# klausondrag/FOSVOS

Hardware: AMD Instinct MI355X
Metric: online fine-tune frames/sec (854x480) (higher is better)
Workload: dtype bf16; 1 GPU; OSVOS_VGG train_online one-shot fine-tune: 1x3x480x854 frame per step, fwd + class-balanced BCE + bwd, fused SGD step every 5 steps (BASELINE.json configs[1]); batch=1, avg_grad_every_n=5, activations=bf16 NHWC, fp32 accumulate, fp32 master weights, parallelism=single GPU

## Files before the change

### fosvos_amd/csrc/common.hpp

```cpp
#pragma once
#include <hip/hip_runtime.h>
#include <stdarg.h>
#include <algorithm>
#include <stdint.h>
#include <stdio.h>
#include <stdlib.h>
#include <string.h>

#include "../../include/fosvos_hip.h"

namespace fosvos {

extern thread_local char g_err[512];

inline int fail(int code, const char *fmt, ...) __attribute__((format(printf, 2, 3)));
inline int fail(int code, const char *fmt, ...) {
    va_list ap;
    va_start(ap, fmt);
    vsnprintf(g_err, sizeof(g_err), fmt, ap);
    va_end(ap);
    return code;
}

#define FOSVOS_HIP_CHECK(expr)                                                                         \
// ... 47 lines not shown
int wgrad_queue_reduce(const float *slabs, const float *bias_part, float *dw, float *db, int S, int S_bias, int64_t E_real,
                       int64_t E_pad, int Co, int Cor, int accumulate, WgradReduceTable *reduce, int device, void *stream);
struct HeadBwdArgs {
    const float *const *side;
    const int *hs, *ws;
    const float *const *filt, *const *filt1;
    const float *dsn_w, *fuse_w, *d_fused;
    const float *const *d_side_out;
    uint16_t *const *d_side;
    float *d_fuse_w, *d_fuse_b, *d_dsn_w, *d_dsn_b;
    int N, H, W, accumulate;
    void *workspace;
    size_t workspace_bytes;
    int device;
    int filt_uniform;
};
int head_bwd_check(const HeadBwdArgs &a);
int head_bwd_scale(const HeadBwdArgs &a, int s, void *stream);
int head_bwd_finish(const HeadBwdArgs &a, void *stream);

}
constexpr int kFosvosVggEvents = 25, kFosvosResnetEvents = 12;
struct fosvos_ctx {
    uint32_t magic;
    int device;
    hipEvent_t vgg_ev[kFosvosVggEvents];
    hipEvent_t resnet_ev[kFosvosResnetEvents];
    bool buckets_recorded;
};
constexpr uint32_t kFosvosCtxMagic = 0x58544346u;
namespace fosvos {
inline int ctx_check(const fosvos_ctx *ctx, const char *who) {
    FOSVOS_REQUIRE(ctx != nullptr, FOSVOS_E_ARG, "%s: null context (fosvos_ctx_create)", who);
    FOSVOS_REQUIRE(ctx->magic == kFosvosCtxMagic, FOSVOS_E_ARG, "%s: not a live fosvos_ctx", who);
    return FOSVOS_OK;
}

#ifdef FOSVOS_LAB_BUILD
inline const char *lab_env(const char *name) { return getenv(name); }
#else
inline const char *lab_env(const char *) { return nullptr; }
#endif
inline int lab_env_int(const char *name, int dflt) {
    const char *e = lab_env(name);
    return e ? atoi(e) : dflt;
}

bool conv_pp_applicable(int N, int H, int W, int in_ch, int out_ch);
int conv_pp_workgroups();
int conv_pp_forward(const uint16_t *x, const uint16_t *w_packed, const float *bias, uint16_t *y, uint16_t *y_pool, int N,
                    int H, int W, int Cin_pad, int Cout, int Co_pad, bool relu, hipStream_t st,
                    const uint8_t *mask_bits = nullptr, uint32_t *codes = nullptr);

bool conv3x3_pool_codes_applicable(int N, int H, int W, int Ci, int Co);

inline int64_t cdiv(int64_t a, int64_t b) { return (a + b - 1) / b; }
inline int roundup(int a, int b) { return (a + b - 1) / b * b; }

typedef uint16_t bf16_t;
typedef __attribute__((ext_vector_type(8))) __bf16 bf16x8;
typedef __attribute__((ext_vector_type(4))) float f32x4;
typedef __attribute__((ext_vector_type(4))) short s16x4;
typedef unsigned int u32x4 __attribute__((__vector_size__(16)));

__device__ __forceinline__ uint16_t f2bf(float f) {
    __bf16 b = (__bf16)f;
    return __builtin_bit_cast(uint16_t, b);
}
__device__ __forceinline__ float bf2f(uint16_t v) { return __uint_as_float(((uint32_t)v) << 16); }
__device__ __forceinline__ uint4 repack8(const float (&f)[8]) {
    uint4 v;
    v.x = __builtin_amdgcn_perm(__float_as_uint(f[1]), __float_as_uint(f[0]), 0x07060302u);
    v.y = __builtin_amdgcn_perm(__float_as_uint(f[3]), __float_as_uint(f[2]), 0x07060302u);
    v.z = __builtin_amdgcn_perm(__float_as_uint(f[5]), __float_as_uint(f[4]), 0x07060302u);
    v.w = __builtin_amdgcn_perm(__float_as_uint(f[7]), __float_as_uint(f[6]), 0x07060302u);
    return v;
}
typedef float fosvos_f32x2 __attribute__((ext_vector_type(2)));
typedef __bf16 fosvos_bf16x2 __attribute__((ext_vector_type(2)));
__device__ __forceinline__ uint32_t pack2bf(float lo, float hi) {
    const fosvos_f32x2 v = {lo, hi};
    return __builtin_bit_cast(uint32_t, __builtin_convertvector(v, fosvos_bf16x2));
}
__device__ __forceinline__ float relu_f(float v) { return __int_as_float(max(__float_as_int(v), 0)); }
__device__ __forceinline__ void unpack8(const uint4 &v, float (&f)[8]) {
    f[0] = __uint_as_float(v.x << 16);
    f[1] = __uint_as_float(v.x & 0xffff0000u);
    f[2] = __uint_as_float(v.y << 16);
    f[3] = __uint_as_float(v.y & 0xffff0000u);
    f[4] = __uint_as_float(v.z << 16);
    f[5] = __uint_as_float(v.z & 0xffff0000u);
    f[6] = __uint_as_float(v.w << 16);
    f[7] = __uint_as_float(v.w & 0xffff0000u);
}
__device__ __forceinline__ uint4 pack8(const float (&f)[8]) {
    uint4 v;
    v.x = pack2bf(f[0], f[1]);
    v.y = pack2bf(f[2], f[3]);
    v.z = pack2bf(f[4], f[5]);
    v.w = pack2bf(f[6], f[7]);
    return v;
}

typedef short fosvos_i16x2 __attribute__((ext_vector_type(2)));
typedef unsigned short fosvos_u16x2 __attribute__((ext_vector_type(2)));
__device__ __forceinline__ uint32_t keep_where_pos_bf16x2(uint32_t f, uint32_t m) {
// ... 92 lines not shown
```

### fosvos_amd/csrc/conv_igemm.hip

```cpp
#include <stdlib.h>

#include "common.hpp"

using namespace fosvos;

namespace {

constexpr unsigned kReluAfterAdd = 0x100u;
constexpr unsigned kSubsample2 = 0x200u;
constexpr unsigned kNoSplitK = 0x400u;

struct ConvArgs {
    const uint16_t *x;
    const uint16_t *w;
    const float *bias;
    const uint16_t *relu_src;
    const uint8_t *relu_bits;
    const uint16_t *addend;
    void *y;
    uint16_t *y_pool;
    const uint16_t *unpool_g;
    int N, H, W, Cin, Cout, Co_pad;
    int tiles_x, tiles_y;
    unsigned flags;
// ... 759 lines not shown
    if ((flags & ~FOSVOS_CONV_RELU) || addend) return false;
    if (dgrad) {
        if (lab_env_int("FOSVOS_PP_DGRAD", 1) == 0 || lab_env_int("FOSVOS_PP", -1) == 0) return false;
    } else {
        static const int mode = lab_env_int("FOSVOS_PP", -1);
        if (mode == 0) return false;
    }
    return conv_pp_applicable(N, H, W, roundup(in_ch, 32), out_ch);
}

int check_common(const void *x, const void *w, const void *y, int N, int H, int W, int in_ch, int out_ch,
                 const char *who) {
    FOSVOS_REQUIRE(x && w && y, FOSVOS_E_ARG, "%s: null pointer", who);
    FOSVOS_REQUIRE(N > 0 && H > 0 && W > 0 && in_ch > 0 && out_ch > 0, FOSVOS_E_SHAPE, "%s: bad shape N=%d H=%d W=%d in=%d out=%d",
                   who, N, H, W, in_ch, out_ch);
    FOSVOS_REQUIRE(out_ch % 16 == 0, FOSVOS_E_SHAPE, "%s: output channels %d not a multiple of 16", who, out_ch);
    FOSVOS_REQUIRE((int64_t)H * W * roundup(in_ch, 32) * 2 < 0x7fffffffLL && (int64_t)H * W * out_ch * 4 < 0x7fffffffLL,
                   FOSVOS_E_SHAPE, "%s: one image exceeds 2^31 bytes", who);
    return FOSVOS_OK;
}
}

extern "C" size_t fosvos_conv3x3_workspace_bytes(int N, int H, int W, int in_ch, int out_ch) {
    if (N <= 0 || H <= 0 || W <= 0 || in_ch <= 0 || out_ch <= 0 || (out_ch % 64 != 0 && out_ch != 16)) return 0;
    return make_plan(N, H, W, in_ch, out_ch).workspace_bytes;
}

extern "C" int fosvos_conv3x3_plan(int N, int H, int W, int in_ch, int out_ch, fosvos_conv3x3_plan_info *out) {
    FOSVOS_REQUIRE(out, FOSVOS_E_ARG, "conv3x3_plan: null output");
    FOSVOS_REQUIRE(N > 0 && H > 0 && W > 0 && in_ch > 0 && out_ch > 0 && (out_ch % 64 == 0 || out_ch == 32 || out_ch == 16),
                   FOSVOS_E_SHAPE, "conv3x3_plan: bad shape N=%d H=%d W=%d in=%d out=%d", N, H, W, in_ch, out_ch);
    const ConvPlan p = make_plan(N, H, W, in_ch, out_ch);
    out->k_splits = p.k_splits;
    out->persistent = 0;
    return with_tile(p.tile, [&](auto t) {
        out->tile_h = t.TH; out->tile_w = t.TW; out->tile_co = t.BN;
        out->workgroups = (int)(cdiv(W, t.TW) * cdiv(H, t.TH) * N * (out_ch / t.BN));
        return FOSVOS_OK;
    });
}

extern "C" int fosvos_conv3x3_fwd_plan(int N, int H, int W, int in_ch, int out_ch, unsigned flags,
                                       fosvos_conv3x3_plan_info *out) {
    if (int rc = fosvos_conv3x3_plan(N, H, W, in_ch, out_ch, out)) return rc;
    if (takes_pp(N, H, W, in_ch, out_ch, flags)) {
        out->tile_h = 8; out->tile_w = 32; out->tile_co = 64;
        out->k_splits = 1;
        out->workgroups = conv_pp_workgroups();
        out->persistent = 1;
    }
    return FOSVOS_OK;
}

extern "C" int fosvos_conv3x3_fwd(const uint16_t *x, const uint16_t *w_packed, const float *bias, void *y, int N, int H,
                                  int W, int Ci, int Co, unsigned flags, void *workspace, size_t workspace_bytes,
                                  int device, void *stream) {
    if (int rc = check_common(x, w_packed, y, N, H, W, Ci, Co, "conv3x3_fwd")) return rc;
    FOSVOS_REQUIRE((flags & ~(FOSVOS_CONV_RELU | FOSVOS_CONV_OUT_F32)) == 0, FOSVOS_E_ARG, "conv3x3_fwd: unknown flags 0x%x", flags);
    FOSVOS_ENTER(device);
    if (takes_pp(N, H, W, Ci, Co, flags))
        return conv_pp_forward(x, w_packed, bias, (uint16_t *)y, nullptr, N, H, W, roundup(Ci, 32), Co, roundup(Co, 16),
                               (flags & FOSVOS_CONV_RELU) != 0, (hipStream_t)stream);
    ConvArgs a = conv_args(x, w_packed, y, N, H, W, Ci, Co);
    a.bias = bias; a.flags = flags;
    return dispatch(a, Ci, workspace, workspace_bytes, (hipStream_t)stream);
}

extern "C" int fosvos_conv3x3_fwd_add(const uint16_t *x, const uint16_t *w_packed, const float *bias,
                                      const uint16_t *addend, void *y, int N, int H, int W, int Ci, int Co,
                                      unsigned flags, void *workspace, size_t workspace_bytes, int device,
                                      void *stream) {
    if (int rc = check_common(x, w_packed, y, N, H, W, Ci, Co, "conv3x3_fwd_add")) return rc;
    FOSVOS_REQUIRE((flags & ~(FOSVOS_CONV_RELU | FOSVOS_CONV_OUT_F32)) == 0, FOSVOS_E_ARG, "conv3x3_fwd_add: unknown flags 0x%x",
                   flags);
    FOSVOS_REQUIRE(Co % 64 == 0 || Co == 32 || (Co == 16 && !addend), FOSVOS_E_SHAPE,
                   "conv3x3_fwd_add: Co=%d must be 32 or a multiple of 64 (16 without an addend)", Co);
    FOSVOS_REQUIRE(!(flags & FOSVOS_CONV_OUT_F32) || (Co == 16 && !addend), FOSVOS_E_ARG,
                   "conv3x3_fwd_add: fp32 output is the 16-channel side_prep form");
    FOSVOS_ENTER(device);
    ConvArgs a = conv_args(x, w_packed, y, N, H, W, Ci, Co);
    a.bias = bias; a.addend = addend;
    a.flags = kNoSplitK | (addend ? ((flags & FOSVOS_CONV_RELU) ? kReluAfterAdd : 0u) : flags);
    return dispatch(a, Ci, workspace, workspace_bytes, (hipStream_t)stream);
}

extern "C" int fosvos_conv3x3_s2_fwd(const uint16_t *x, const uint16_t *w_packed, const float *bias, uint16_t *y, int N,
                                     int H, int W, int Ci, int Co, unsigned flags, void *workspace, size_t workspace_bytes,
                                     int device, void *stream) {
    if (int rc = check_common(x, w_packed, y, N, H, W, Ci, Co, "conv3x3_s2_fwd")) return rc;
    FOSVOS_REQUIRE((flags & ~FOSVOS_CONV_RELU) == 0, FOSVOS_E_ARG, "conv3x3_s2_fwd: unknown flags 0x%x", flags);
    FOSVOS_REQUIRE(Co % 64 == 0 || Co == 32, FOSVOS_E_SHAPE, "conv3x3_s2_fwd: Co=%d must be 32 or a multiple of 64", Co);
    FOSVOS_ENTER(device);
    ConvArgs a = conv_args(x, w_packed, y, N, H, W, Ci, Co);
    a.bias = bias; a.flags = flags | kSubsample2 | kNoSplitK;
    return dispatch(a, Ci, workspace, workspace_bytes, (hipStream_t)stream);
}

extern "C" int fosvos_conv3x3_fwd_pool(const uint16_t *x, const uint16_t *w_packed, const float *bias, uint16_t *y,
                                       uint16_t *y_pool, int N, int H, int W, int Ci, int Co, unsigned flags,
                                       void *workspace, size_t workspace_bytes, int device, void *stream) {
    if (int rc = check_common(x, w_packed, y, N, H, W, Ci, Co, "conv3x3_fwd_pool")) return rc;
    FOSVOS_REQUIRE(y_pool, FOSVOS_E_ARG, "conv3x3_fwd_pool: null pooled output");
    FOSVOS_REQUIRE((flags & ~FOSVOS_CONV_RELU) == 0, FOSVOS_E_ARG, "conv3x3_fwd_pool: unknown flags 0x%x", flags);
    FOSVOS_REQUIRE(Co % 64 == 0, FOSVOS_E_SHAPE, "conv3x3_fwd_pool: Co=%d must be a multiple of 64", Co);
    if ((flags & FOSVOS_CONV_RELU) && takes_pp(N, H, W, Ci, Co, flags)) {
        FOSVOS_ENTER(device);
        return conv_pp_forward(x, w_packed, bias, y, y_pool, N, H, W, roundup(Ci, 32), Co, roundup(Co, 16), true,
                               (hipStream_t)stream);
    }
    if (make_plan(N, H, W, Ci, Co).k_splits > 1) {
        if (int rc = fosvos_conv3x3_fwd(x, w_packed, bias, y, N, H, W, Ci, Co, flags, workspace, workspace_bytes, device, stream))
            return rc;
        return fosvos_maxpool2x2_ceil_fwd(y, y_pool, N, H, W, Co, device, stream);
    }
    FOSVOS_ENTER(device);
// ... 77 lines not shown
```

### fosvos_amd/fosvos_hip/__init__.py

```python
from __future__ import annotations

import ctypes
import os
import threading
from ctypes import POINTER, c_char_p, c_float, c_int, c_int64, c_size_t, c_uint, c_void_p

_HERE = os.path.dirname(os.path.abspath(__file__))
PKG_ROOT = os.path.dirname(_HERE)
LIB_PATH = os.environ.get("FOSVOS_HIP_LIB") or os.path.join(PKG_ROOT, "lib", "libfosvos_hip.so")
HEADER_PATH = os.path.join(os.path.dirname(PKG_ROOT), "include", "fosvos_hip.h")

ABI_VERSION = 34
CONV_RELU = 1
CONV_OUT_F32 = 2
VGG_COMPACT_STAGE1 = 1


class FosvosHipError(RuntimeError):
    pass


class SgdEntry(ctypes.Structure):
    _fields_ = [("param", c_void_p), ("grad", c_void_p), ("momentum_buf", c_void_p), ("numel", c_int64),
                ("lr", c_float), ("weight_decay", c_float)]
# ... 24 lines not shown
    _fields_ = [("total", c_size_t), ("stage_h", c_int * 5), ("stage_w", c_int * 5),
                ("act", _Z13), ("gact", _Z13), ("act_bytes", _Z13),
                ("pooled", _Z4), ("gpooled", _Z4), ("pooled_bytes", _Z4),
                ("side", _Z4), ("side_bytes", _Z4), ("dside", _Z4), ("dside_bytes", _Z4),
                ("bits0", c_size_t), ("bits0_bytes", c_size_t),
                ("ws", c_size_t), ("ws_bytes", c_size_t), ("hws", c_size_t), ("hws_bytes", c_size_t),
                ("wsa_conv", _Z13), ("wsa_conv_bytes", _Z13), ("wsa_side", _Z4), ("wsa_side_bytes", _Z4)]


class Conv3x3PlanInfo(ctypes.Structure):
    _fields_ = [("tile_h", c_int), ("tile_w", c_int), ("tile_co", c_int), ("k_splits", c_int), ("workgroups", c_int),
                ("persistent", c_int)]


class Conv2dPlanInfo(ctypes.Structure):
    _fields_ = [("cob", c_int), ("threads", c_int), ("slices", c_int), ("workgroups", c_int), ("mfma_frag_blocks", c_int),
                ("mfma_workgroups", c_int)]


class ProfileRecord(ctypes.Structure):
    _fields_ = [("name", ctypes.c_char * 96), ("launches", c_int), ("ms", ctypes.c_double), ("flops", ctypes.c_double)]


class PackEntry(ctypes.Structure):
    _fields_ = [("w", c_void_p), ("w_fwd", c_void_p), ("w_dgrad", c_void_p), ("Co", c_int), ("Ci", c_int)]



class Conv2dDesc(ctypes.Structure):
    _fields_ = [("w_packed", c_void_p), ("bias", c_void_p), ("Ci", c_int), ("Co", c_int), ("k", c_int), ("stride", c_int),
                ("kind", c_int)]


class ResnetBlock(ctypes.Structure):
    _fields_ = [("conv", Conv2dDesc * 3), ("n_convs", c_int), ("has_down", c_int), ("down", Conv2dDesc)]


class ResnetNet(ctypes.Structure):
    _fields_ = [("first_w", c_void_p), ("first_b", c_void_p), ("first_co", c_int), ("first_fp32_math", c_int), ("first_unfused", c_int),
                ("blocks_per_stage", c_int * 4),
                ("blocks", POINTER(ResnetBlock)), ("side", Conv2dDesc * 4), ("filt", c_void_p * 4),
                ("filt1", c_void_p * 4), ("stride", c_int * 4), ("dsn_w", c_void_p), ("dsn_b", c_void_p),
                ("fuse_b", c_void_p)]

SIGNATURES = {
    "fosvos_abi_version": (c_int, []),
    "fosvos_last_error": (c_char_p, []),
    "fosvos_build_arch": (c_char_p, []),
    "fosvos_ctx_create": (c_int, [c_int, POINTER(c_void_p)]),
    "fosvos_ctx_destroy": (c_int, [c_void_p]),
    "fosvos_ctx_device": (c_int, [c_void_p]),
    "fosvos_conv3x3_plan": (c_int, [c_int, c_int, c_int, c_int, c_int, POINTER(Conv3x3PlanInfo)]),
    "fosvos_conv3x3_fwd_plan": (c_int, [c_int, c_int, c_int, c_int, c_int, ctypes.c_uint, POINTER(Conv3x3PlanInfo)]),
    "fosvos_conv3x3_first_plan": (c_int, [c_int, c_int, c_int, POINTER(c_int), POINTER(c_int)]),
    "fosvos_nchw_f32_to_nhwc_bf16": (c_int, [c_void_p, c_void_p, c_int, c_int, c_int, c_int, c_int, c_int, c_void_p]),
    "fosvos_nhwc_bf16_to_nchw_f32": (c_int, [c_void_p, c_void_p, c_int, c_int, c_int, c_int, c_int, c_int, c_void_p]),
    "fosvos_nhwc_f32_to_nchw_f32": (c_int, [c_void_p, c_void_p, c_int, c_int, c_int, c_int, c_int, c_void_p]),
    "fosvos_nchw_f32_to_nhwc_f32": (c_int, [c_void_p, c_void_p, c_int, c_int, c_int, c_int, c_int, c_void_p]),
    "fosvos_pack_conv3x3_weights": (c_int, [c_void_p, c_int, c_int, c_void_p, c_void_p, c_int, c_void_p]),
    "fosvos_packed_weight_elems": (c_size_t, [c_int, c_int]),
    "fosvos_pack_conv3x3_weights_multi": (c_int, [POINTER(PackEntry), c_int, c_int, c_void_p]),
    "fosvos_conv3x3_first_fwd": (c_int, [c_void_p, c_void_p, c_void_p, c_void_p, c_void_p, c_int, c_int, c_int, c_int, c_int,
                                         c_void_p]),
    "fosvos_conv3x3_dgrad_bits": (c_int, [c_void_p, c_void_p, c_void_p, c_void_p, c_void_p, c_int, c_int, c_int, c_int,
                                          c_int, c_void_p, c_size_t, c_int, c_void_p]),
    "fosvos_conv3x3_dgrad_unpool": (c_int, [c_void_p, c_void_p, c_void_p, c_void_p, c_void_p, c_int, c_int, c_int, c_int,
                                            c_int, c_void_p, c_size_t, c_int, c_void_p]),
    "fosvos_conv3x3_first_wgrad": (c_int, [c_void_p, c_void_p, c_void_p, c_void_p, c_int, c_int, c_int, c_int,
                                           c_void_p, c_size_t, c_int, c_void_p]),
    "fosvos_conv3x3_first_wgrad_workspace_bytes": (c_size_t, [c_int, c_int, c_int, c_int]),
    "fosvos_conv3x3_fwd": (c_int, [c_void_p, c_void_p, c_void_p, c_void_p, c_int, c_int, c_int, c_int, c_int, c_uint,
                                   c_void_p, c_size_t, c_int, c_void_p]),
    "fosvos_conv3x3_fwd_pool": (c_int, [c_void_p, c_void_p, c_void_p, c_void_p, c_void_p, c_int, c_int, c_int, c_int,
                                        c_int, c_uint, c_void_p, c_size_t, c_int, c_void_p]),
    "fosvos_conv3x3_workspace_bytes": (c_size_t, [c_int, c_int, c_int, c_int, c_int]),
    "fosvos_conv3x3_dgrad": (c_int, [c_void_p, c_void_p, c_void_p, c_void_p, c_void_p, c_int, c_int, c_int, c_int,
                                     c_int, c_void_p, c_size_t, c_int, c_void_p]),
    "fosvos_conv3x3_wgrad": (c_int, [c_void_p, c_void_p, c_void_p, c_void_p, c_int, c_int, c_int, c_int, c_int, c_int,
                                     c_void_p, c_size_t, c_int, c_void_p]),
    "fosvos_conv3x3_wgrad_slabs": (c_int, [c_void_p, c_void_p, c_int, c_int, c_int, c_int, c_int, c_int, c_void_p, c_size_t,
                                           c_int, c_void_p]),
    "fosvos_conv3x3_wgrad_reduce": (c_int, [c_void_p, c_void_p, c_int, c_int, c_int, c_int, c_int, c_int, c_void_p,
                                            c_size_t, c_int, c_void_p]),
    "fosvos_conv3x3_wgrad_workspace_bytes": (c_size_t, [c_int, c_int, c_int, c_int, c_int]),
    "fosvos_maxpool2x2_ceil_fwd": (c_int, [c_void_p, c_void_p, c_int, c_int, c_int, c_int, c_int, c_void_p]),
    "fosvos_maxpool2x2_ceil_bwd": (c_int, [c_void_p, c_void_p, c_void_p, c_int, c_int, c_int, c_int, c_int, c_int,
                                           c_void_p]),
    "fosvos_head_fwd": (c_int, [POINTER(c_void_p), POINTER(c_int), POINTER(c_int), POINTER(c_void_p),
                                POINTER(c_void_p), c_void_p, c_void_p, c_void_p, c_void_p, c_void_p,
                                POINTER(c_void_p), c_int, c_int, c_int, c_int, c_int, c_void_p]),
    "fosvos_head_bwd": (c_int, [POINTER(c_void_p), POINTER(c_int), POINTER(c_int), POINTER(c_void_p),
                                POINTER(c_void_p), c_void_p, c_void_p, c_void_p, POINTER(c_void_p),
                                POINTER(c_void_p), c_void_p, c_void_p, c_void_p, c_void_p, c_int, c_int, c_int, c_int,
                                c_void_p, c_size_t, c_int, c_void_p]),
    "fosvos_head_bwd_workspace_bytes": (c_size_t, [c_int, c_int, c_int]),
    "fosvos_cbce_loss": (c_int, [c_void_p, c_void_p, c_int64, c_int, c_float, c_void_p, c_void_p, c_void_p, c_size_t,
                                 c_int, c_void_p]),
    "fosvos_cbce_workspace_bytes": (c_size_t, [c_int64]),
    "fosvos_cbce_loss_frames": (c_int, [c_void_p, c_void_p, c_int64, c_int, c_int, c_float, c_void_p, c_void_p, c_void_p,
                                        c_size_t, c_int, c_void_p]),
    "fosvos_cbce_loss_frames_parts": (c_int, [c_void_p, c_void_p, c_int64, c_int, c_int, c_float, c_void_p, c_void_p,
                                              c_void_p, c_size_t, c_int, c_int, c_void_p]),
    "fosvos_cbce_multi_workspace_bytes": (c_size_t, [c_int64, c_int, c_int]),
    "fosvos_cbce_loss_frames_multi": (c_int, [POINTER(c_void_p), c_void_p, c_int64, c_int, c_int, c_int, POINTER(c_float),
                                              c_void_p, POINTER(c_void_p), c_void_p, c_size_t, c_int, c_int, c_void_p]),
    "fosvos_cbce_loss_batch_counts": (c_int, [c_void_p, c_void_p, c_int64, c_int, c_float, c_void_p, c_void_p, c_void_p,
# ... 195 lines not shown
```

### fosvos_amd/fosvos_hip/ops.py

```python
from __future__ import annotations

import ctypes
import math
from typing import List, Optional, Sequence, Tuple

import torch

from . import CONV_OUT_F32, CONV_RELU, check, int_array4, lib, limits, ptr_array4

_BF16 = torch.bfloat16
_F32 = torch.float32


def _need(t: torch.Tensor, dtype, what: str, dtype_error=TypeError) -> torch.Tensor:
    if not t.is_cuda:
        raise RuntimeError(f"{what}: tensor must live on the GPU (the HIP path has no CPU fallback)")
    if t.dtype != dtype:
        raise dtype_error(f"{what}: expected {dtype}, got {t.dtype}")
    if not t.is_contiguous():
        raise ValueError(f"{what}: tensor must be contiguous")
    return t


def _ctx(t: torch.Tensor) -> Tuple[int, int]:
# ... 139 lines not shown
        if (kh, kw) != (3, 3) or w.device != ws[0].device:
            raise ValueError("pack_conv3x3_weights_multi: 3x3 kernels on one device only")
        fwd = torch.empty(L.fosvos_packed_weight_elems(co, ci), dtype=_BF16, device=w.device)
        dgr = torch.empty(L.fosvos_packed_weight_elems(ci, co), dtype=_BF16, device=w.device)
        arr[i].w, arr[i].w_fwd, arr[i].w_dgrad, arr[i].Co, arr[i].Ci = w.data_ptr(), fwd.data_ptr(), dgr.data_ptr(), co, ci
        out.append((fwd, dgr))
        nbytes += w.numel() * 4 + 2 * (fwd.numel() + dgr.numel())
    _launch("pack_conv3x3_weights_multi", ws[0], arr, len(ws), record="pack_weights", nbytes=nbytes)
    return out


def conv3x3_first_fwd(frame: torch.Tensor, w: torch.Tensor, b: torch.Tensor, want_bits: bool = False):
    _need(frame, _F32, "conv3x3_first_fwd frame"); _need(w, _F32, "conv3x3_first_fwd weight"); _need(b, _F32, "conv3x3_first_fwd bias")
    n, c, h, wd = frame.shape
    if c != 3 or tuple(w.shape[1:]) != (3, 3, 3):
        raise ValueError("conv3x3_first_fwd: expects a 3-channel frame and [Co,3,3,3] weights")
    co = w.shape[0]
    y = torch.empty((n, h, wd, co), dtype=_BF16, device=frame.device)
    bits = torch.empty((n, h, wd, co // 8), dtype=torch.uint8, device=frame.device) if want_bits else None
    _launch("conv3x3_first_fwd", frame, frame.data_ptr(), w.data_ptr(), b.data_ptr(), y.data_ptr(), _p(bits), n, h, wd, co,
            record="conv1_1_fwd", flops=2.0 * n * h * wd * 27 * co, nbytes=n * h * wd * (12 + 2 * co))
    return (y, bits) if want_bits else y


def conv3x3_first_wgrad(frame: torch.Tensor, dy: torch.Tensor) -> Tuple[torch.Tensor, torch.Tensor]:
    _need(frame, _F32, "conv3x3_first_wgrad frame"); _need(dy, _BF16, "conv3x3_first_wgrad dy")
    n, c, h, wd = frame.shape
    co = dy.shape[3]
    if tuple(dy.shape[:3]) != (n, h, wd):
        raise ValueError("conv3x3_first_wgrad: dy shape mismatch")
    L = lib()
    dw = torch.empty((co, 3, 3, 3), dtype=_F32, device=frame.device)
    db = torch.empty((co,), dtype=_F32, device=frame.device)
    ws, wsn = _WS.get(L.fosvos_conv3x3_first_wgrad_workspace_bytes(n, h, wd, co), frame.device)
    _launch("conv3x3_first_wgrad", frame, frame.data_ptr(), dy.data_ptr(), dw.data_ptr(), db.data_ptr(), n, h, wd, co, ws, wsn,
            record="conv1_1_wgrad", flops=2.0 * n * h * wd * 27 * co, nbytes=n * h * wd * (12 + 2 * co))
    return dw, db


def conv3x3_plan(n: int, h: int, w: int, in_ch: int, out_ch: int) -> dict:
    from . import Conv3x3PlanInfo
    info = Conv3x3PlanInfo()
    check(lib().fosvos_conv3x3_plan(n, h, w, in_ch, out_ch, ctypes.byref(info)), "conv3x3_plan")
    return {"tile": (info.tile_h, info.tile_w, info.tile_co), "k_splits": info.k_splits, "workgroups": info.workgroups,
            "persistent": bool(info.persistent)}


def conv3x3_fwd_plan(n: int, h: int, w: int, in_ch: int, out_ch: int, relu: bool = True) -> dict:
    from . import Conv3x3PlanInfo
    info = Conv3x3PlanInfo()
    check(lib().fosvos_conv3x3_fwd_plan(n, h, w, in_ch, out_ch, CONV_RELU if relu else 0, ctypes.byref(info)), "conv3x3_fwd_plan")
    return {"tile": (info.tile_h, info.tile_w, info.tile_co), "k_splits": info.k_splits, "workgroups": info.workgroups,
            "persistent": bool(info.persistent)}


def vgg_arena_layout(n: int, h: int, w: int) -> dict:
    from . import VggArenaLayout
    info = VggArenaLayout()
    check(lib().fosvos_vgg_arena_layout(n, h, w, ctypes.byref(info)), "vgg_arena_layout")
    out = {}
    for name, _ in VggArenaLayout._fields_:
        v = getattr(info, name)
        out[name] = list(v) if isinstance(v, ctypes.Array) else int(v)
    return out


def conv3x3_first_plan(n: int, h: int, w: int) -> Tuple[int, int]:
    tiles, wgs = ctypes.c_int(), ctypes.c_int()
    check(lib().fosvos_conv3x3_first_plan(n, h, w, ctypes.byref(tiles), ctypes.byref(wgs)), "conv3x3_first_plan")
    return tiles.value, wgs.value


def conv3x3_fwd(x: torch.Tensor, w_packed: torch.Tensor, bias: Optional[torch.Tensor], ci: int, co: int,
                relu: bool = True, out_f32: bool = False) -> torch.Tensor:
    _need(x, _BF16, "conv3x3_fwd x"); _need(w_packed, _BF16, "conv3x3_fwd packed weight")
    n, h, wd, cx = x.shape
    if cx != _ru(ci, 32):
        raise ValueError(f"conv3x3_fwd: x has {cx} channels, expected {_ru(ci, 32)} (Ci={ci} padded to 32)")
    L = lib()
    if w_packed.numel() != L.fosvos_packed_weight_elems(co, ci):
        raise ValueError("conv3x3_fwd: packed weight size does not match (Co, Ci)")
    if bias is not None:
        _need(bias, _F32, "conv3x3_fwd bias")
        if bias.numel() != co:
            raise ValueError("conv3x3_fwd: bias size")
    y = torch.empty((n, h, wd, co), dtype=_F32 if out_f32 else _BF16, device=x.device)
    flags = (CONV_RELU if relu else 0) | (CONV_OUT_F32 if out_f32 else 0)
    ws, wsn = _WS.get(L.fosvos_conv3x3_workspace_bytes(n, h, wd, ci, co), x.device)
    _launch("conv3x3_fwd", x, x.data_ptr(), w_packed.data_ptr(), _p(bias), y.data_ptr(), n, h, wd, ci, co, flags, ws, wsn,
            flops=2.0 * n * h * wd * 9 * ci * co, nbytes=n * h * wd * (2 * cx + (4 if out_f32 else 2) * co) + 2 * 9 * ci * co)
    return y


def conv3x3_fwd_pool(x: torch.Tensor, w_packed: torch.Tensor, bias: Optional[torch.Tensor], ci: int, co: int,
                     relu: bool = True) -> Tuple[torch.Tensor, torch.Tensor]:
    _need(x, _BF16, "conv3x3_fwd_pool x"); _need(w_packed, _BF16, "conv3x3_fwd_pool packed weight")
    n, h, wd, cx = x.shape
    if cx != _ru(ci, 32):
        raise ValueError(f"conv3x3_fwd_pool: x has {cx} channels, expected {_ru(ci, 32)}")
    L = lib()
    if w_packed.numel() != L.fosvos_packed_weight_elems(co, ci):
        raise ValueError("conv3x3_fwd_pool: packed weight size does not match (Co, Ci)")
    if bias is not None:
        _need(bias, _F32, "conv3x3_fwd_pool bias")
    y = torch.empty((n, h, wd, co), dtype=_BF16, device=x.device)
    yp = torch.empty((n, (h + 1) // 2, (wd + 1) // 2, co), dtype=_BF16, device=x.device)
# ... 1351 lines not shown
```

### include/fosvos_hip.h

```cpp
#ifndef FOSVOS_HIP_H
#define FOSVOS_HIP_H

#include <stddef.h>
#include <stdint.h>

#ifdef __cplusplus
extern "C" {
#endif

#define FOSVOS_ABI_VERSION 34

#define FOSVOS_OK 0
#define FOSVOS_E_SHAPE (-1)
#define FOSVOS_E_ARG (-2)
#define FOSVOS_E_WORKSPACE (-3)
#define FOSVOS_E_HIP (-4)

#define FOSVOS_CONV_RELU 1u
#define FOSVOS_CONV_OUT_F32 2u
#define FOSVOS_CONV_FP32_MATH 4u

int fosvos_abi_version(void);

typedef struct fosvos_profile_record {
// ... 24 lines not shown
    size_t act[13], gact[13], act_bytes[13];
    size_t pooled[4], gpooled[4], pooled_bytes[4];
    size_t side[4], side_bytes[4];
    size_t dside[4], dside_bytes[4];
    size_t bits0, bits0_bytes;
    size_t ws, ws_bytes, hws, hws_bytes;
    size_t wsa_conv[13], wsa_conv_bytes[13], wsa_side[4], wsa_side_bytes[4];
} fosvos_vgg_arena_layout_info;
int fosvos_vgg_arena_layout(int N, int H, int W, fosvos_vgg_arena_layout_info *out);

int fosvos_pack_conv3x3_weights(const float *w_oihw, int Co, int Ci, uint16_t *w_fwd, uint16_t *w_dgrad,
                                int device, void *stream);
size_t fosvos_packed_weight_elems(int out_ch, int in_ch);

typedef struct fosvos_pack_entry {
    const float *w;
    uint16_t *w_fwd, *w_dgrad;
    int Co, Ci;
} fosvos_pack_entry;
int fosvos_pack_conv3x3_weights_multi(const fosvos_pack_entry *entries, int n, int device, void *stream);

int fosvos_conv3x3_first_fwd(const float *frame, const float *w_oihw, const float *bias, uint16_t *y, uint8_t *relu_bits,
                             int N, int H, int W, int Co, int device, void *stream);
int fosvos_conv3x3_first_plan(int N, int H, int W, int *tiles, int *workgroups);
int fosvos_conv3x3_first_wgrad(const float *frame, const uint16_t *dy, float *dw_oihw, float *dbias, int N, int H,
                               int W, int Co, void *workspace, size_t workspace_bytes, int device, void *stream);
size_t fosvos_conv3x3_first_wgrad_workspace_bytes(int N, int H, int W, int Co);

int fosvos_conv3x3_fwd(const uint16_t *x, const uint16_t *w_packed, const float *bias, void *y, int N, int H, int W,
                       int Ci, int Co, unsigned flags, void *workspace, size_t workspace_bytes, int device,
                       void *stream);

int fosvos_conv3x3_s2_fwd(const uint16_t *x, const uint16_t *w_packed, const float *bias, uint16_t *y, int N, int H, int W,
                          int Ci, int Co, unsigned flags, void *workspace, size_t workspace_bytes, int device, void *stream);
int fosvos_conv3x3_fwd_add(const uint16_t *x, const uint16_t *w_packed, const float *bias, const uint16_t *addend,
                           void *y, int N, int H, int W, int Ci, int Co, unsigned flags, void *workspace,
                           size_t workspace_bytes, int device, void *stream);
int fosvos_conv3x3_fwd_pool(const uint16_t *x, const uint16_t *w_packed, const float *bias, uint16_t *y,
                            uint16_t *y_pool, int N, int H, int W, int Ci, int Co, unsigned flags, void *workspace,
                            size_t workspace_bytes, int device, void *stream);
int fosvos_conv3x3_fwd_pool_codes(const uint16_t *x, const uint16_t *w_packed, const float *bias, uint16_t *y_pool,
                                  uint32_t *codes, int N, int H, int W, int Ci, int Co, unsigned flags, int device,
                                  void *stream);
size_t fosvos_conv3x3_pool_codes_bytes(int N, int H, int W, int C);
size_t fosvos_conv3x3_workspace_bytes(int N, int H, int W, int in_ch, int out_ch);
typedef struct fosvos_conv3x3_plan_info {
    int tile_h, tile_w, tile_co;
    int k_splits;
    int workgroups;
    int persistent;
} fosvos_conv3x3_plan_info;
int fosvos_conv3x3_plan(int N, int H, int W, int in_ch, int out_ch, fosvos_conv3x3_plan_info *out);
int fosvos_conv3x3_fwd_plan(int N, int H, int W, int in_ch, int out_ch, unsigned flags, fosvos_conv3x3_plan_info *out);
int fosvos_conv3x3_dgrad(const uint16_t *dy, const uint16_t *w_dgrad_packed, const uint16_t *relu_src,
                         const uint16_t *addend, uint16_t *dx, int N, int H, int W, int Ci, int Co, void *workspace,
                         size_t workspace_bytes, int device, void *stream);
int fosvos_conv3x3_dgrad_bits(const uint16_t *dy, const uint16_t *w_dgrad_packed, const uint8_t *relu_bits,
                              const uint16_t *addend, uint16_t *dx, int N, int H, int W, int Ci, int Co, void *workspace,
                              size_t workspace_bytes, int device, void *stream);
int fosvos_conv3x3_dgrad_unpool(const uint16_t *dy, const uint16_t *w_dgrad_packed, const uint16_t *x,
                                const uint16_t *d_pooled, uint16_t *dx, int N, int H, int W, int Ci, int Co,
                                void *workspace, size_t workspace_bytes, int device, void *stream);
int fosvos_conv3x3_wgrad(const uint16_t *x, const uint16_t *dy, float *dw_oihw, float *dbias, int N, int H, int W,
                         int Ci, int Co, int accumulate, void *workspace, size_t workspace_bytes, int device,
                         void *stream);
size_t fosvos_conv3x3_wgrad_workspace_bytes(int N, int H, int W, int Ci, int Co);
int fosvos_conv3x3_wgrad_slabs(const uint16_t *x, const uint16_t *dy, int with_bias, int N, int H, int W, int Ci, int Co,
                               void *workspace, size_t workspace_bytes, int device, void *stream);
int fosvos_conv3x3_wgrad_reduce(float *dw_oihw, float *dbias, int N, int H, int W, int Ci, int Co, int accumulate,
                                void *workspace, size_t workspace_bytes, int device, void *stream);

int fosvos_maxpool2x2_ceil_fwd(const uint16_t *x, uint16_t *y, int N, int H, int W, int C, int device, void *stream);
int fosvos_maxpool2x2_ceil_bwd(const uint16_t *x, const uint16_t *dy, uint16_t *dx, int N, int H, int W, int C,
                               int relu_mask, int device, void *stream);
int fosvos_maxpool2x2_ceil_bwd_codes(const uint32_t *codes, const uint16_t *dy, uint16_t *dx, int N, int H, int W, int C,
                                     int device, void *stream);

int fosvos_head_fwd(const float *const side[4], const int hs[4], const int ws[4], const float *const filt[4],
                    const float *const filt1[4], const float *dsn_w , const float *dsn_b ,
                    const float *fuse_w , const float *fuse_b , float *fused,
                    float *const side_out[4] , int N, int H, int W, int filt_uniform, int device,
                    void *stream);
int fosvos_head_bwd(const float *const side[4], const int hs[4], const int ws[4], const float *const filt[4],
                    const float *const filt1[4], const float *dsn_w, const float *fuse_w, const float *d_fused,
                    const float *const d_side_out[4], uint16_t *const d_side[4], float *d_fuse_w, float *d_fuse_b,
                    float *d_dsn_w, float *d_dsn_b, int N, int H, int W, int filt_uniform ,
                    void *workspace, size_t workspace_bytes, int device, void *stream);
size_t fosvos_head_bwd_workspace_bytes(int N, int H, int W);

int fosvos_cbce_loss(const float *logits, const float *label, int64_t numel, int size_average, float grad_scale,
                     float *loss_out, float *grad, void *workspace, size_t workspace_bytes, int device,
                     void *stream);
size_t fosvos_cbce_workspace_bytes(int64_t numel);
int fosvos_cbce_loss_frames(const float *logits, const float *label, int64_t frame_numel, int n_frames, int size_average,
                            float grad_scale, float *loss_out, float *grad, void *workspace, size_t workspace_bytes,
                            int device, void *stream);
#define FOSVOS_CBCE_COUNT 1
#define FOSVOS_CBCE_LOSS 2
#define FOSVOS_CBCE_FINISH 4
int fosvos_cbce_loss_frames_parts(const float *logits, const float *label, int64_t frame_numel, int n_frames,
                                  int size_average, float grad_scale, float *loss_out, float *grad, void *workspace,
                                  size_t workspace_bytes, int parts, int device, void *stream);
#define FOSVOS_CBCE_MAX_MAPS 8
size_t fosvos_cbce_multi_workspace_bytes(int64_t frame_numel, int n_frames, int n_maps);
int fosvos_cbce_loss_frames_multi(const float *const *logits, const float *label, int64_t frame_numel, int n_frames,
                                  int n_maps, int size_average, const float *map_scale, float *loss_out, float *const *grad,
// ... 227 lines not shown
```

Baseline: 1232 frames/s.

## Add persistent LDS-resident side-conv kernel for 16-channel fp32 output convs

Adds a dedicated persistent kernel for the 3x3 side-output convs with 16 output channels and fp32 output. All weights stay resident in LDS, and input halos are double-buffered with direct buffer-to-LDS DMA. Tiles are statically split across XCD groups, and the split-K partial sums are reduced in registers, so the igemm path's partial workspace and its reduce step are no longer needed. LDS use is capped so that a workgroup of the other branch's igemm can co-reside, at the cost of a large new hand-scheduled kernel with inline asm.

```diff
diff --git a/fosvos_amd/csrc/common.hpp b/fosvos_amd/csrc/common.hpp
--- a/fosvos_amd/csrc/common.hpp
+++ b/fosvos_amd/csrc/common.hpp
@@ -123,6 +123,10 @@
                     int H, int W, int Cin_pad, int Cout, int Co_pad, bool relu, hipStream_t st,
                     const uint8_t *mask_bits = nullptr, uint32_t *codes = nullptr);
 
+int conv_side_workgroups(int N, int H, int W, int Cin_pad, int igemm_k_splits);
+int conv_side_forward(const uint16_t *x, const uint16_t *w_packed, const float *bias, float *y, int N, int H, int W,
+                      int Cin_pad, bool relu, int chunks_per_split, int workgroups, hipStream_t st);
+
 bool conv3x3_pool_codes_applicable(int N, int H, int W, int Ci, int Co);
 
 inline int64_t cdiv(int64_t a, int64_t b) { return (a + b - 1) / b; }
diff --git a/fosvos_amd/csrc/conv_igemm.hip b/fosvos_amd/csrc/conv_igemm.hip
--- a/fosvos_amd/csrc/conv_igemm.hip
+++ b/fosvos_amd/csrc/conv_igemm.hip
@@ -835,6 +835,16 @@
     return FOSVOS_OK;
 }
 
+extern "C" int fosvos_conv3x3_side_plan(int N, int H, int W, int Ci, int Co, unsigned flags, int *workgroups) {
+    FOSVOS_REQUIRE(workgroups, FOSVOS_E_ARG, "conv3x3_side_plan: null output");
+    FOSVOS_REQUIRE(N > 0 && H > 0 && W > 0 && Ci > 0, FOSVOS_E_SHAPE, "conv3x3_side_plan: bad shape N=%d H=%d W=%d Ci=%d", N, H, W, Ci);
+    FOSVOS_REQUIRE(Co == 16, FOSVOS_E_SHAPE, "conv3x3_side_plan: Co=%d (the side form has 16 output channels)", Co);
+    FOSVOS_REQUIRE((flags & FOSVOS_CONV_OUT_F32) && !(flags & ~(FOSVOS_CONV_RELU | FOSVOS_CONV_OUT_F32)), FOSVOS_E_ARG,
+                   "conv3x3_side_plan: flags 0x%x (the side form is FOSVOS_CONV_OUT_F32, optionally with FOSVOS_CONV_RELU)", flags);
+    *workgroups = conv_side_workgroups(N, H, W, roundup(Ci, 32), make_plan(N, H, W, Ci, Co).k_splits);
+    return FOSVOS_OK;
+}
+
 extern "C" int fosvos_conv3x3_fwd(const uint16_t *x, const uint16_t *w_packed, const float *bias, void *y, int N, int H,
                                   int W, int Ci, int Co, unsigned flags, void *workspace, size_t workspace_bytes,
                                   int device, void *stream) {
@@ -844,6 +854,12 @@
     if (takes_pp(N, H, W, Ci, Co, flags))
         return conv_pp_forward(x, w_packed, bias, (uint16_t *)y, nullptr, N, H, W, roundup(Ci, 32), Co, roundup(Co, 16),
                                (flags & FOSVOS_CONV_RELU) != 0, (hipStream_t)stream);
+    if (Co == 16 && (flags & FOSVOS_CONV_OUT_F32)) {
+        const ConvPlan plan = make_plan(N, H, W, Ci, Co);
+        if (const int wgs = conv_side_workgroups(N, H, W, roundup(Ci, 32), plan.k_splits))
+            return conv_side_forward(x, w_packed, bias, (float *)y, N, H, W, roundup(Ci, 32), (flags & FOSVOS_CONV_RELU) != 0,
+                                     plan.chunks_per_split, wgs, (hipStream_t)stream);
+    }
     ConvArgs a = conv_args(x, w_packed, y, N, H, W, Ci, Co);
     a.bias = bias; a.flags = flags;
     return dispatch(a, Ci, workspace, workspace_bytes, (hipStream_t)stream);
diff --git a/fosvos_amd/csrc/conv_side.hip b/fosvos_amd/csrc/conv_side.hip
--- /dev/null
+++ b/fosvos_amd/csrc/conv_side.hip
@@ -0,0 +1,276 @@
+#include "common.hpp"
+
+using namespace fosvos;
+
+namespace fosvos {
+namespace side {
+
+struct Args {
+    const uint16_t *x;
+    const uint16_t *w;
+    const float *bias;
+    float *y;
+    int N, H, W, Cin;
+    int tiles_x, tiles_y, n_tiles;
+    int chunks_per_split;
+    int relu;
+};
+
+template <int WR_, int WC_, int R_, int MAX_NC_>
+struct Cfg {
+    static constexpr int WR = WR_, WC = WC_, R = R_, MAX_NC = MAX_NC_;
+    static constexpr int TH = WR * R, TW = WC * 16;
+    static constexpr int HALO_W = TW + 2, HALO_H = TH + 2, NPIX = HALO_W * HALO_H;
+    static constexpr int A_PIECES = (NPIX * 4 + 63) / 64;
+    static constexpr int A_BYTES = A_PIECES * 1024;
+    static constexpr int A_IT = (A_PIECES + 3) / 4;
+    static constexpr int W_CHUNK = 9 * 1024;
+    static constexpr int LDS_MAX = MAX_NC * W_CHUNK + 2 * A_BYTES;
+    static_assert(WR * WC == 4, "four waves");
+    static_assert(A_IT <= R + 2, "one DMA piece per halo row");
+    static_assert(LDS_MAX <= 96 * 1024, "a side-conv workgroup leaves room for an igemm workgroup of the other chain");
+};
+using CfgWide = Cfg<2, 2, 4, 4>;
+using CfgNarrow = Cfg<4, 1, 2, 8>;
+
+#pragma clang diagnostic push
+#pragma clang diagnostic ignored "-Winline-asm"
+__device__ __forceinline__ void dma16(const __amdgpu_buffer_rsrc_t rsrc, unsigned lds_dst, unsigned voff, unsigned soff) {
+    asm volatile("s_mov_b32 m0, %0\n\ts_nop 4\n\tbuffer_load_dwordx4 %1, %2, %3 offen lds"
+                 :: "s"(lds_dst), "v"(voff), "s"(rsrc), "s"(soff) : "memory", "m0");
+}
+__device__ __forceinline__ void wait_all() { asm volatile("s_waitcnt vmcnt(0) lgkmcnt(0)" ::: "memory"); }
+__device__ __forceinline__ void step_barrier() {
+    asm volatile("" ::: "memory");
+    __builtin_amdgcn_s_barrier();
+    asm volatile("" ::: "memory");
+}
+#pragma clang diagnostic pop
+
+typedef __attribute__((address_space(3))) void lds_void;
+typedef __attribute__((address_space(3))) const uint4 *lds_u4_ptr;
+
+struct TileIt {
+    int idx, n, ty, tx;
+    int d_n, d_ty, d_tx, stride;
+    int tiles_x, tiles_y, end;
+    __device__ __forceinline__ void init(int first, int stride_, int tiles_x_, int tiles_y_, int end_) {
+        tiles_x = tiles_x_; tiles_y = tiles_y_; end = end_; stride = stride_;
+        idx = first;
+        const int per_img = tiles_x * tiles_y;
+        n = first / per_img;
+        const int r = first - n * per_img;
+        ty = r / tiles_x;
+        tx = r - ty * tiles_x;
+        d_n = stride / per_img;
+        const int rs = stride - d_n * per_img;
+        d_ty = rs / tiles_x;
+        d_tx = rs - d_ty * tiles_x;
+    }
+    __device__ __forceinline__ void next() {
+        idx += stride;
+        tx += d_tx;
+        const int cx = tx >= tiles_x;
+        tx -= cx ? tiles_x : 0;
+        ty += d_ty + cx;
+        const int cy = ty >= tiles_y;
+        ty -= cy ? tiles_y : 0;
+        n += d_n + cy;
+    }
+    __device__ __forceinline__ bool valid() const { return idx < end; }
+};
+
+template <class C>
+__global__ __launch_bounds__(256) __attribute__((amdgpu_waves_per_eu(4, 4))) void k_conv3x3_side(const Args a) {
+    extern __shared__ __attribute__((aligned(16))) char smem_side[];
+    constexpr int R = C::R;
+    const unsigned lds0 = __builtin_amdgcn_readfirstlane((unsigned)(size_t)(lds_void *)smem_side);
+    const int tid = threadIdx.x, lane = tid & 63;
+    const int wave = __builtin_amdgcn_readfirstlane(tid >> 6);
+    const int wr = wave / C::WC, wc = wave % C::WC;
+    const int cl = lane & 15, kq = lane >> 4;
+    const int H = a.H, W = a.W, Cin = a.Cin;
+    const int NC = Cin >> 5;
+    const unsigned lds_a = lds0 + NC * C::W_CHUNK;
+
+    const int b = blockIdx.x, S = gridDim.x >> 3;
+    const int xcd = b & 7, j = b >> 3;
+    const int t_begin = (int)(((int64_t)xcd * a.n_tiles) >> 3), t_end = (int)(((int64_t)(xcd + 1) * a.n_tiles) >> 3);
+    const int span = t_end - t_begin;
+    if (span <= j) return;
+    const int K = ((span - j + S - 1) / S) * NC;
+    TileIt cur, ldt;
+    cur.init(t_begin + j, S, a.tiles_x, a.tiles_y, t_end);
+    ldt = cur;
+
+    int ld_c = 0, ld_y0 = 0, ld_x0 = 0;
+    unsigned ld_dst = 0;
+    bool ld_on = false;
+    __amdgpu_buffer_rsrc_t ld_rsrc = __builtin_amdgcn_make_buffer_rsrc(const_cast<uint16_t *>(a.x), 0, 0, 0x00020000);
+    auto ld_open = [&](int step) {
+        ld_on = step < K;
+        if (!ld_on) return;
+        ld_rsrc = __builtin_amdgcn_make_buffer_rsrc(const_cast<uint16_t *>(a.x) + (int64_t)ldt.n * H * W * Cin, 0, H * W * Cin * 2,
+                                                    0x00020000);
+        ld_y0 = ldt.ty * C::TH; ld_x0 = ldt.tx * C::TW;
+        ld_dst = lds_a + (step & 1) * C::A_BYTES;
+    };
+    auto ld_piece = [&](int i) {
+        const int pc = wave + 4 * i;
+        if (!ld_on || pc >= C::A_PIECES) return;
+        const int P = pc * 16 + (lane >> 2), s4 = lane & 3;
+        const int hy = P / C::HALO_W, hx = P - hy * C::HALO_W;
+        const int gy = ld_y0 + hy - 1, gx = ld_x0 + hx - 1;
+        const bool ok = P < C::NPIX && (unsigned)gy < (unsigned)H && (unsigned)gx < (unsigned)W;
+        const unsigned voff = ok ? ((unsigned)(gy * W + gx) * (unsigned)(Cin * 2) + (unsigned)((s4 ^ ((P >> 1) & 2)) << 4)) : 0x80000000u;
+        dma16(ld_rsrc, ld_dst + pc * 1024, voff, (unsigned)(ld_c * 64));
+    };
+    auto ld_advance = [&]() {
+        if (++ld_c == NC) { ld_c = 0; ldt.next(); }
+    };
+
+    {
+        const auto w_rsrc = __builtin_amdgcn_make_buffer_rsrc(const_cast<uint16_t *>(a.w), 0, NC * C::W_CHUNK, 0x00020000);
+        for (int p = wave; p < NC * 9; p += 4) dma16(w_rsrc, lds0 + p * 1024, (unsigned)(lane * 16), (unsigned)(p * 1024));
+    }
+    ld_open(0);
+#pragma unroll
+    for (int i = 0; i < C::A_IT; ++i) ld_piece(i);
+    ld_advance();
+
+    unsigned a_sw[R + 2][3];
+#pragma unroll
+    for (int h = 0; h < R + 2; ++h)
+#pragma unroll
+        for (int kx = 0; kx < 3; ++kx) {
+            const int P = (wr * R + h) * C::HALO_W + wc * 16 + kx + cl;
+            a_sw[h][kx] = (unsigned)(P * 64 + ((kq ^ ((P >> 1) & 2)) << 4));
+        }
+    const unsigned w_frag0 = lds0 + lane * 16;
+
+    float4 bias = make_float4(0.f, 0.f, 0.f, 0.f);
+    if (a.bias) bias = *reinterpret_cast<const float4 *>(a.bias + kq * 4);
+
+    f32x4 acc[R], total[R];
+#pragma unroll
+    for (int r = 0; r < R; ++r) acc[r] = total[r] = f32x4{0.f, 0.f, 0.f, 0.f};
+    int cp_c = 0, cp_s = 0;
+    bool first_sum = true;
+    int dn_n = 0, dn_y0 = 0, dn_x0 = 0;
+    bool st_pending = false;
+    auto store_tile = [&]() {
+        const auto y_rsrc = __builtin_amdgcn_make_buffer_rsrc(a.y + (int64_t)dn_n * H * W * 16, 0, H * W * 64, 0x00020000);
+#pragma unroll
+        for (int r = 0; r < R; ++r) {
+            const int gy = dn_y0 + wr * R + r, gx = dn_x0 + wc * 16 + cl;
+            const unsigned off = (gy < H && gx < W) ? (unsigned)(((gy * W + gx) * 16 + kq * 4) * 4) : 0x80000000u;
+            __builtin_amdgcn_raw_buffer_store_b128(__builtin_bit_cast(u32x4, total[r]), y_rsrc, off, 0, 0);
+        }
+        st_pending = false;
+    };
+
+    wait_all();
+    step_barrier();
+
+    for (int k = 0; k < K; ++k) {
+        if (st_pending) store_tile();
+        ld_open(k + 1);
+        const unsigned abuf = lds_a + (k & 1) * C::A_BYTES;
+        const unsigned wbuf = w_frag0 + cp_c * C::W_CHUNK;
+        bf16x8 wf[9], af[3];
+#pragma unroll
+        for (int t = 0; t < 9; ++t) wf[t] = __builtin_bit_cast(bf16x8, *(lds_u4_ptr)(size_t)(wbuf + t * 1024));
+#pragma unroll
+        for (int h = 0; h < R + 2; ++h) {
+#pragma unroll
+            for (int kx = 0; kx < 3; ++kx) af[kx] = __builtin_bit_cast(bf16x8, *(lds_u4_ptr)(size_t)(abuf + a_sw[h][kx]));
+            if (h < C::A_IT) ld_piece(h);
+#pragma unroll
+            for (int kx = 0; kx < 3; ++kx)
+#pragma unroll
+                for (int ky = 0; ky < 3; ++ky) {
+                    const int r = h - ky;
+                    if (r >= 0 && r < R)
+                        acc[r] = __builtin_amdgcn_mfma_f32_16x16x32_bf16(wf[ky * 3 + kx], af[kx], acc[r], 0, 0, 0);
+                }
+        }
+        ld_advance();
+        ++cp_c; ++cp_s;
+        if (cp_s == a.chunks_per_split || cp_c == NC) {
+#pragma unroll
+            for (int r = 0; r < R; ++r) {
+                total[r] = first_sum ? acc[r] : total[r] + acc[r];
+                acc[r] = f32x4{0.f, 0.f, 0.f, 0.f};
+            }
+            first_sum = false;
+            cp_s = 0;
+        }
+        if (cp_c == NC) {
+#pragma unroll
+            for (int r = 0; r < R; ++r) {
+                f32x4 v = total[r];
+                v[0] += bias.x; v[1] += bias.y; v[2] += bias.z; v[3] += bias.w;
+                if (a.relu) { v[0] = relu_f(v[0]); v[1] = relu_f(v[1]); v[2] = relu_f(v[2]); v[3] = relu_f(v[3]); }
+                total[r] = v;
+            }
+            dn_n = cur.n; dn_y0 = cur.ty * C::TH; dn_x0 = cur.tx * C::TW;
+            st_pending = true;
+            first_sum = true;
+            cp_c = 0;
+            cur.next();
+        }
+        wait_all();
+        step_barrier();
+    }
+    if (st_pending) store_tile();
+}
+
+template <class C>
+int launch(const Args &a0, int wgs, hipStream_t st) {
+    Args a = a0;
+    a.tiles_x = (int)cdiv(a.W, C::TW);
+    a.tiles_y = (int)cdiv(a.H, C::TH);
+    a.n_tiles = a.tiles_x * a.tiles_y * a.N;
+    const int lds = (a.Cin >> 5) * C::W_CHUNK + 2 * C::A_BYTES;
+    static bool once[64];
+    int dev = 0;
+    FOSVOS_HIP_CHECK(hipGetDevice(&dev));
+    if (dev >= 0 && dev < 64 && !once[dev]) {
+        FOSVOS_HIP_CHECK(hipFuncSetAttribute(reinterpret_cast<const void *>(k_conv3x3_side<C>),
+                                             hipFuncAttributeMaxDynamicSharedMemorySize, C::LDS_MAX));
+        once[dev] = true;
+    }
+    FOSVOS_PROF("k_conv3x3_side", st, 2.0 * a.N * a.H * a.W * 9.0 * a.Cin * 16);
+    hipLaunchKernelGGL(k_conv3x3_side<C>, dim3((unsigned)wgs), dim3(256), lds, st, a);
+    FOSVOS_LAUNCH_CHECK();
+    return FOSVOS_OK;
+}
+
+constexpr int kMaxWorkgroups = 512;
+
+}
+
+int conv_side_workgroups(int N, int H, int W, int Cin_pad, int igemm_k_splits) {
+    if (N <= 0 || H <= 0 || W <= 0 || Cin_pad <= 0 || Cin_pad % 32 != 0 || Cin_pad > 32 * side::CfgNarrow::MAX_NC) return 0;
+    const bool wide = Cin_pad <= 32 * side::CfgWide::MAX_NC;
+    const int mode = lab_env_int("FOSVOS_SIDE", -1);
+    if (mode == 0 || (mode != 1 && !wide && igemm_k_splits <= 1)) return 0;
+    const int64_t tiles = wide ? cdiv(H, side::CfgWide::TH) * cdiv(W, side::CfgWide::TW) * N
+                               : cdiv(H, side::CfgNarrow::TH) * cdiv(W, side::CfgNarrow::TW) * N;
+    if (tiles > 0x3fffffff) return 0;
+    const int cap = wide ? side::kMaxWorkgroups : side::kMaxWorkgroups / 2;
+    return (int)std::min<int64_t>(cap, roundup((int)tiles, 8));
+}
+
+int conv_side_forward(const uint16_t *x, const uint16_t *w_packed, const float *bias, float *y, int N, int H, int W,
+                      int Cin_pad, bool relu, int chunks_per_split, int workgroups, hipStream_t st) {
+    side::Args a{};
+    a.x = x; a.w = w_packed; a.bias = bias; a.y = y;
+    a.N = N; a.H = H; a.W = W; a.Cin = Cin_pad;
+    a.chunks_per_split = chunks_per_split;
+    a.relu = relu ? 1 : 0;
+    if (Cin_pad <= 32 * side::CfgWide::MAX_NC) return side::launch<side::CfgWide>(a, workgroups, st);
+    return side::launch<side::CfgNarrow>(a, workgroups, st);
+}
+
+}
diff --git a/fosvos_amd/fosvos_hip/__init__.py b/fosvos_amd/fosvos_hip/__init__.py
--- a/fosvos_amd/fosvos_hip/__init__.py
+++ b/fosvos_amd/fosvos_hip/__init__.py
@@ -100,6 +100,7 @@
     "fosvos_ctx_device": (c_int, [c_void_p]),
     "fosvos_conv3x3_plan": (c_int, [c_int, c_int, c_int, c_int, c_int, POINTER(Conv3x3PlanInfo)]),
     "fosvos_conv3x3_fwd_plan": (c_int, [c_int, c_int, c_int, c_int, c_int, ctypes.c_uint, POINTER(Conv3x3PlanInfo)]),
+    "fosvos_conv3x3_side_plan": (c_int, [c_int, c_int, c_int, c_int, c_int, ctypes.c_uint, POINTER(c_int)]),
     "fosvos_conv3x3_first_plan": (c_int, [c_int, c_int, c_int, POINTER(c_int), POINTER(c_int)]),
     "fosvos_nchw_f32_to_nhwc_bf16": (c_int, [c_void_p, c_void_p, c_int, c_int, c_int, c_int, c_int, c_int, c_void_p]),
     "fosvos_nhwc_bf16_to_nchw_f32": (c_int, [c_void_p, c_void_p, c_int, c_int, c_int, c_int, c_int, c_int, c_void_p]),
diff --git a/fosvos_amd/fosvos_hip/ops.py b/fosvos_amd/fosvos_hip/ops.py
--- a/fosvos_amd/fosvos_hip/ops.py
+++ b/fosvos_amd/fosvos_hip/ops.py
@@ -215,6 +215,13 @@
     check(lib().fosvos_conv3x3_fwd_plan(n, h, w, in_ch, out_ch, CONV_RELU if relu else 0, ctypes.byref(info)), "conv3x3_fwd_plan")
     return {"tile": (info.tile_h, info.tile_w, info.tile_co), "k_splits": info.k_splits, "workgroups": info.workgroups,
             "persistent": bool(info.persistent)}
+
+
+def conv3x3_side_plan(n: int, h: int, w: int, ci: int, co: int = 16, relu: bool = False, out_f32: bool = True) -> int:
+    wgs = ctypes.c_int()
+    flags = (CONV_RELU if relu else 0) | (CONV_OUT_F32 if out_f32 else 0)
+    check(lib().fosvos_conv3x3_side_plan(n, h, w, ci, co, flags, ctypes.byref(wgs)), "conv3x3_side_plan")
+    return wgs.value
 
 
 def vgg_arena_layout(n: int, h: int, w: int) -> dict:
diff --git a/include/fosvos_hip.h b/include/fosvos_hip.h
--- a/include/fosvos_hip.h
+++ b/include/fosvos_hip.h
@@ -100,6 +100,7 @@
 } fosvos_conv3x3_plan_info;
 int fosvos_conv3x3_plan(int N, int H, int W, int in_ch, int out_ch, fosvos_conv3x3_plan_info *out);
 int fosvos_conv3x3_fwd_plan(int N, int H, int W, int in_ch, int out_ch, unsigned flags, fosvos_conv3x3_plan_info *out);
+int fosvos_conv3x3_side_plan(int N, int H, int W, int Ci, int Co, unsigned flags, int *workgroups);
 int fosvos_conv3x3_dgrad(const uint16_t *dy, const uint16_t *w_dgrad_packed, const uint16_t *relu_src,
                          const uint16_t *addend, uint16_t *dx, int N, int H, int W, int Ci, int Co, void *workspace,
                          size_t workspace_bytes, int device, void *stream);
```

Result: no change. 1232 frames/s (-0.1%).
